# tingyu-c/TW-invoice-unet-ocr-llm

Hardware: AMD Instinct MI355X
Metric: invoice masks/sec at 512x512 bs256, 1/2/4/8 MI355X; IoU vs CPU ref (higher is better)
Workload: dtype bf16+fp16

## Files before the change

### tw-invoice-unet-ocr-llm_amd/csrc/unet_capi.cpp

```cpp
#include "unet_internal.h"
#include "unet_score.h"
#include "unet_loss.h"
#include "unet_head.h"
#include "../../include/unet_mi355x.h"

#include <dlfcn.h>

#include <algorithm>
#include <cmath>
#include <cstdio>
#include <cstdlib>
#include <cstring>
#include <list>
#include <map>
#include <string>
#include <thread>
#include <tuple>
#include <vector>

using namespace unet;

namespace {

thread_local std::string g_err;
// ... 87 lines not shown
  std::vector<void*> allocs;
  std::list<std::pair<std::tuple<int, int, int, int>, ResampleStore>> resample;
  uint8_t* pp_tmp = nullptr;
  size_t pp_tmp_bytes = 0;
  std::string labels[UNET_NUM_LAUNCHES];
  float thr_logit[kMaxClasses];
  hipEvent_t done = nullptr;
  hipStream_t last_stream = nullptr;
  bool pending = false;
  bool capturing = false;
  void* comm = nullptr;
  unsigned long long generation = 1;
  int ksplit_max = 32;
  int f32x3 = 0;
  int ksplit_force[21] = {};
  void* part = nullptr;
  int* box_sync = nullptr;
  int box_sync_n = 0;
  void* score = nullptr;
  size_t score_bytes = 0;
  void* loss = nullptr;
  size_t loss_bytes = 0;
  void* head = nullptr;
  size_t head_bytes = 0;
};

struct unet_graph {
  unet_handle* h = nullptr;
  hipGraph_t graph = nullptr;
  hipGraphExec_t exec = nullptr;
// ... 52 lines not shown
    {C3A, EPI_STORE, 2, B_(cat3), 512, B_(tA), 256},
    {C3B, EPI_STORE, 2, B_(tA), 256, B_(tB), 256},
    {19, EPI_UPSCATTER, 2, B_(tB), 256, B_(cat2), 256, 0, {}, 0, "u2", 128},
    {C2A, EPI_STORE, 1, B_(cat2), 256, B_(tA), 128},
    {C2B, EPI_STORE, 1, B_(tA), 128, B_(tB), 128, 0, {}, 0, "c7", 128},
    {20, EPI_UPSCATTER, 1, B_(tB), 128, B_(cat1), 128, 0, {}, 0, "u1", 64},
    {C1A, EPI_STORE, 0, B_(cat1), 128, B_(tA), 64, 0, {}, 0, "c8a", 64},
    {C1B, EPI_HEAD, 0, B_(tA), 64}};
#undef B_
static_assert(sizeof kLaunches / sizeof kLaunches[0] == UNET_NUM_LAUNCHES - 1, "one row per launch slot after the first");
const int kRingCfg[17] = {
    CFG_RING8_FUSED_IN,
    CFG_RING8_R128, CFG_RING8_R128, CFG_RING8_R128, CFG_RING8_R128, CFG_RING8_R128, CFG_RING8_R128,
    CFG_RING8_R128, CFG_RING8_R128, CFG_RING8_R128, CFG_RING8_R128, CFG_RING8_R128, CFG_RING8_R128,
    CFG_RING8_R128, CFG_RING8_R128,
    CFG_RING8_R64_T9, CFG_RING8_R64_WS};
const int kHaloCfg[17] = {
    CFG_HALO_R64_W8,
    CFG_HALO_R128, CFG_HALO_R128, CFG_HALO_R128, CFG_HALO_R64_W4, CFG_HALO_R128, CFG_HALO_R64_W4,
    CFG_HALO_R128, CFG_HALO_R128, CFG_HALO_R128, CFG_HALO_R128, CFG_HALO_R128, CFG_HALO_R128,
    CFG_HALO_R128, CFG_HALO_R128,
    CFG_HALO_R64_W4, CFG_HALO_R64_W8};

DType level_dtype(int dtype, int level) {
  switch (dtype) {
    case UNET_DTYPE_F32: case UNET_DTYPE_F32_EXACT: return DType::F32;
    case UNET_DTYPE_F16: return DType::F16;
    case UNET_DTYPE_MIXED: return level <= 1 ? DType::F16 : DType::BF16;
    default: return DType::BF16;
  }
}
// ... 70 lines not shown
  if (row.id >= 17) {
    if (!(row.id == 20 && h->fuse_up1)) st.L = &up_layer(h, row.id - 17, N);
    return st;
  }
  st.L = &h->L[row.id];
  if (row.id == C2B && h->fuse_up1) {
    st.r.epi = EPI_UPFUSE;
    st.r.out = nullptr;
    st.r.ldo = 0;
    st.r.out2 = &Buffers::cat1;
    st.r.ldo2 = 128;
  }
  if (row.id == D1B && cfg_fused_in(st.L->cfg)) st.r.id = -1;
  return st;
}
Split step_split(const unet_handle* h, const Step& st, int N, int H, int W) {
  return layer_split(h, st.r.id, *st.L, st.r.epi, N, H >> st.r.level, W >> st.r.level);
}

size_t split_bytes(const unet_handle* h, int N, int H, int W) {
  size_t m = 0;
  for (const Launch& row : kLaunches) {
    const Step st = resolve(h, row, N);
    const int ks = st.L ? step_split(h, st, N, H, W).ks : 1;
    if (ks > 1) m = std::max(m, (size_t)ks * N * (H >> row.level) * (W >> row.level) * st.L->ctot * 4);
  }
  return m;
}

Buffers plan(const unet_handle* h, int N, int H, int W) {
// ... 448 lines not shown
std::string layer_label(const Layer& L, int epi, Split sp = Split{}) {
  char buf[160];
  int cfg = L.cfg;
  if (sp.ks == 1 && sp.rows && cfg == CFG_TRING_R256) cfg = CFG_TRING_R128;
  if (sp.ks > 1) {
    Layer P = L;
    P.dto = P.dtq = L.dt;
    std::string part = layer_label(P, EPI_PARTIAL, Split{1, sp.rows});
    std::snprintf(buf, sizeof buf, " + splitk_reduce_kernel<%s, %s, %d>", tname(L.dto),
                  tname(epi == EPI_POOL ? L.dtq : L.dto), epi);
    return part + buf;
  }
  if (cfg_is_tring(cfg)) {
    std::snprintf(buf, sizeof buf, "convT_ring_kernel<%s, 8, %d, %d, %s>", tname(L.dt), cfg == CFG_TRING_R256 ? 4 : 3,
                  cfg == CFG_TRING_R256 ? 2 : 1, tname(L.dto));
  } else if (cfg_is_ring8(cfg)) {
    const int wst = cfg == CFG_RING8_R64_WS || cfg == CFG_RING8_FUSED_IN;
    const int rows = (sp.rows && cfg == CFG_RING8_R128) ? sp.rows : cfg_rows(cfg);
    std::snprintf(buf, sizeof buf, "conv3x3_ring8_kernel<%s, %d, %d, %d, %d, %d, %s, %s, %d, 0>", tname(L.dt),
                  rows / 16, ring_ns(cfg), epi, ring_tps(cfg), wst, tname(L.dto),
                  tname(epi == EPI_POOL ? L.dtq : L.dto), cfg == CFG_RING8_FUSED_IN ? 1 : 0);
  } else if (cfg_is_ring(cfg)) {
    std::snprintf(buf, sizeof buf, "conv3x3_ring_kernel<%s, 1, 4, %d, %d, %d, %d, %d, %s, %s, %d, %d>", tname(L.dt),
                  cfg_rows(cfg) / 16, ring_ns(cfg), epi, ring_tps(cfg), cfg == CFG_RING_FUSED_IN ? 1 : 0,
                  tname(L.dto), tname(epi == EPI_POOL ? L.dtq : L.dto), cfg_tile_h(cfg), cfg_tile_w(cfg));
  } else if (L.x3 == 3 || L.x3 == 4) {
    std::snprintf(buf, sizeof buf, L.x3 == 3 ? "conv3x3_x3s_kernel<%d>" : "conv3x3_x3w_kernel<%d>", epi);
  } else {
    const int wpx = cfg == CFG_HALO_R64_W8 ? 8 : 4, tc = cfg == CFG_HALO_R128 ? 8 : 4,
              ns = L.x3 == 2 ? 2 : cfg == CFG_HALO_R128 ? 2 : 3;
// ... 1 lines not shown
                  L.taps == 9 ? 3 : 1, epi, L.x3);
  }
  return buf;
}

void build_labels_at(const unet_handle* h, int N, int H, int W, std::string (&out)[UNET_NUM_LAUNCHES]) {
  const int C = h->cfg.n_channels;
  char buf[96];
  const DType t0 = h->L[D1B].dt;
  std::snprintf(buf, sizeof buf, t0 == DType::F32 ? "first_conv_kernel<%s, %d>" : "first_conv_mfma_kernel<%s, %d>",
                tname(t0), C);
  out[0] = cfg_fused_in(h->L[D1B].cfg) ? std::string("x_to_px4_kernel<") + tname(t0) + ">" : buf;
  int i = 1;
  for (const Launch& row : kLaunches) {
    const Step st = resolve(h, row, N);
    out[i++] = st.L ? layer_label(*st.L, st.r.epi, step_split(h, st, N, H, W)) : std::string();
  }
}
void build_labels(unet_handle* h) { build_labels_at(h, 0, 0, 0, h->labels); }

template <typename F>
void parse_pairs(const char* list, F each) {
  const std::string o(list ? list : "");
  for (size_t pos = 0, end; pos < o.size(); pos = end + 1) {
    end = std::min(o.find(',', pos), o.size());
    const std::string item = o.substr(pos, end - pos);
    const size_t colon = item.find(':');
    if (colon != std::string::npos)
      each(std::atoi(item.substr(0, colon).c_str()), std::atoi(item.substr(colon + 1).c_str()), item);
  }
}
void parse_overrides(const char* ov, int n, int* cfg_out, bool (*ok)(int)) {
  parse_pairs(ov, [&](int li, int c, const std::string& item) {
    if (li >= 0 && li < n && c >= 0 && c < cfg_limit() && ok(c)) cfg_out[li] = c;
    else std::fprintf(stderr, "unet_mi355x: ignoring configuration override '%s'\n", item.c_str());
  });
}

struct NcclId { char internal[UNET_COMM_ID_BYTES]; };
struct Rccl {
  void* lib = nullptr;
  int (*get_unique_id)(NcclId*) = nullptr;
  int (*comm_init_rank)(void**, int, NcclId, int) = nullptr;
  int (*all_gather)(const void*, void*, size_t, int, void*, hipStream_t) = nullptr;
  int (*comm_destroy)(void*) = nullptr;
  const char* (*error_string)(int) = nullptr;
};
const Rccl* rccl() {
  static Rccl r;
// ... 77 lines not shown
  for (const Launch& row : kLaunches) {
    if (row.id >= 17) continue;
    const int i = row.id;
    const bool pool = row.epi == EPI_POOL;
    Layer& L = h->L[i];
    L.cin = kLayerCh[i][0];
    L.cout = L.ctot = kLayerCh[i][1];
    L.taps = 9;
    L.dt = L.dto = level_dtype(cfg->dtype, row.level);
    L.dtq = level_dtype(cfg->dtype, row.level + 1);
    int c = cfgs[i];
    const bool ring = cfg_is_ring(c);
    if (cfg_fused_in(c) && (i != D1B || f32))
      c = cfg_is_ring8(c) ? (L.cout == 64 ? CFG_RING8_R64_T9 : CFG_RING8_R128)
                          : (L.cout == 64 ? CFG_RING_R64_T3 : CFG_RING_R128);
    if (c == CFG_RING8_R64_WS && (L.cin != 64 || f32)) c = L.cout == 64 ? CFG_RING8_R64_T9 : CFG_RING8_R128;
    if (c == CFG_RING8_R128 && (L.cout == 64 || f32)) c = CFG_RING8_R64_T9;
    if (c == CFG_RING_R64_W12 && f32) c = CFG_RING_R64_T3;
    if (cfg_rows(c) > L.cout || (i == C1B && cfg_rows(c) != 64))
      c = ring ? CFG_RING_R64_T3 : CFG_HALO_R64_W8;
    if (cfg_is_halo(c) && (L.dto != L.dt || (pool && L.dtq != L.dt))) c = L.cout == 64 || pool ? CFG_RING_R64_T3 : CFG_RING_R128;
    if (c == CFG_RING_R128 && pool) c = CFG_RING_R64_T3;
    if (h->f32x3 && f32) {
#ifndef UNET_X3_ONCE_MIN_CIN
#define UNET_X3_ONCE_MIN_CIN 128
#endif
      const bool once = h->f32x3 == 2 && L.cout % 128 == 0 && L.cin >= UNET_X3_ONCE_MIN_CIN && i != C1B;
      const bool wide = h->f32x3 == 2 && i == C1B;
      c = once ? CFG_HALO_R128 : wide ? CFG_HALO_X3W : CFG_HALO_R64_W4;
      L.x3 = once ? 3 : wide ? 4 : 2;
// ... 16 lines not shown
      U.x3 = 1;
      if (h->f32x3 == 2) {
        h->Us[i] = U;
        h->Us[i].cfg = CFG_HALO_R64_W4;
        h->Us[i].x3 = 2;
      }
    }
  }
  {
    const char* fz = std::getenv("UNET_MI355X_FUSE_UP1");
    const Layer &c2b = h->L[C2B], &u1 = h->U[3];
    h->fuse_up1 = !(fz && fz[0] == '0') && !f32 && (c2b.cfg == CFG_RING_R128 || c2b.cfg == CFG_RING8_R128) &&
                  u1.dt == c2b.dt && u1.dto == c2b.dto;
  }
  if (const char* ks = std::getenv("UNET_MI355X_KSPLIT")) h->ksplit_max = std::atoi(ks);
  parse_pairs(std::getenv("UNET_MI355X_KSPLIT_FORCE"), [&](int li, int ks, const std::string&) {
    if (li >= 0 && li < 21) h->ksplit_force[li] = ks;
  });
  build_labels(h);
  DeviceGuard g(cfg->device);
  const int rc = init_handle(h);
  if (rc) { delete h; return rc; }
  *out = h;
  return UNET_OK;
}

int unet_load_weights(unet_handle* h, const unet_tensor_view* t, int n) {
  if (!h || (!t && n)) return fail(UNET_EINVAL, "null argument");
  SD sd;
  for (int i = 0; i < n; ++i) {
// ... 130 lines not shown
  a.bias = L.b;
  a.zero = h->zero;
  a.out = out;
  a.out2 = out2;
  a.head_w = h->head_w;
  a.head_b = h->head_b;
  a.logits = logits;
  a.masks = static_cast<uint8_t*>(masks);
  a.N = N; a.H = H; a.W = W;
  a.Cin = L.cin; a.ldi = ldi;
  a.Ctot = L.ctot; a.Cout = L.cout;
  a.ldo = ldo; a.out_off = out_off; a.ldo2 = ldo2;
  a.ncls = h->cfg.n_classes;
  a.mask_kind = mask_kind;
  a.x3 = L.x3;
  if (epi == EPI_UPFUSE) {
    a.wgt = h->wf_c2b;
    a.bias2 = h->U[3].b;
  }
  if (cfg_fused_in(L.cfg)) {
    a.x0 = x0;
    a.w0p = h->w0r;
    a.b0 = h->b0;
    a.c0 = h->cfg.n_channels;
  }
  for (int i = 0; i < kMaxClasses; ++i) a.thr_logit[i] = h->thr_logit[i];
  a.tiles_x = (W + cfg_tile_w(L.cfg) - 1) / cfg_tile_w(L.cfg);
  a.tiles_y = (H + cfg_tile_h(L.cfg) - 1) / cfg_tile_h(L.cfg);
  a.n_ct = L.ctot / cfg_rows(L.cfg);
  const Split sp = layer_split(h, id, L, epi, N, H, W);
  int cfg = L.cfg;
  if (sp.ks == 1 && sp.rows) {
    a.src_br = cfg_rows(L.cfg);
    a.n_ct = L.ctot / sp.rows;
    if (L.cfg == CFG_TRING_R256) cfg = CFG_TRING_R128;
  }
  if (sp.ks > 1) {
    a.part = static_cast<float*>(h->part);
    a.ksplit = sp.ks;
    if (sp.rows) {
      a.src_br = cfg_rows(L.cfg);
      a.n_ct = L.ctot / sp.rows;
    }
    hipError_t e = launch_igemm(L.dt, L.dt, L.dt, L.cfg, L.taps, EPI_PARTIAL, a, s);
    if (e == hipSuccess) e = launch_splitk_reduce(L.dto, epi == EPI_POOL ? L.dtq : L.dto, epi, a, s);
    if (e != hipSuccess) return fail(UNET_EHIP, std::string("split-K igemm launch: ") + hipGetErrorString(e));
// ... 863 lines not shown
```

### tw-invoice-unet-ocr-llm_amd/csrc/unet_internal.h

```cpp
#pragma once
#include <hip/hip_runtime.h>
#include <cstdint>
#include <cstddef>

namespace unet {

enum class DType : int { F32 = 0, BF16 = 1, F16 = 2 };

inline size_t dtype_size(DType t) { return t == DType::F32 ? 4 : 2; }

enum Epi : int {
  EPI_STORE = 0,
  EPI_POOL = 1,
  EPI_HEAD = 2,
  EPI_UPSCATTER = 3,
  EPI_UPFUSE = 4,
  EPI_PARTIAL = 5
};

enum MaskKind : int { MASK_NONE = 0, MASK_U8 = 1, MASK_BITS = 2 };

constexpr int kMaxClasses = 4;

struct IgemmArgs {
// ... 12 lines not shown
  int Ctot;
  int Cout;
  int ldo, out_off, ldo2;
  int ncls, mask_kind;
  float thr_logit[kMaxClasses];
  int tiles_x, tiles_y, n_ct;
  const void* x0;
  const void* w0p;
  const float* b0;
  int c0;
  const float* bias2;
  float* part;
  int ksplit;
  int src_br;
  int x3;
};

struct FirstConvArgs {
  const float* x;
  const float* w;
  const void* wp;
  const float* b;
  void* out;
  int N, C, H, W;
};

__host__ __device__ constexpr int first_tap(int s) { return (int)((0xF8F5F2764310ull >> (4 * s)) & 15); }
__host__ __device__ constexpr int first_tap_addr(int s) { return (int)((0x885522764310ull >> (4 * s)) & 15); }

enum Cfg : int {
  CFG_HALO_R64_W4 = 0,
  CFG_HALO_R64_W8 = 1,
  CFG_HALO_R128 = 2,
  CFG_RING_R128 = 3,
  CFG_RING_R64_T3 = 4,
  CFG_RING_FUSED_IN = 5,
  CFG_TRING_R128 = 6,
  CFG_TRING_R256 = 7,
  CFG_RING8_R128 = 8,
  CFG_RING8_R64_T9 = 9,
  CFG_RING8_R64_WS = 10,
  CFG_RING8_FUSED_IN = 11,
  CFG_RING_R64_W12 = 12,
  CFG_HALO_X3W = 13,
  CFG_COUNT = 14
};
int cfg_rows(int cfg);
bool cfg_is_halo(int cfg);
bool cfg_is_ring(int cfg);
int ring_ns(int cfg);
int ring_tps(int cfg);
int cfg_tile_w(int cfg);
int cfg_tile_h(int cfg);
bool cfg_is_ring8(int cfg);
bool cfg_fused_in(int cfg);
bool cfg_is_tring(int cfg);
int cfg_limit();

hipError_t launch_igemm(DType t, DType to, DType tq, int cfg, int taps, int epi, const IgemmArgs& a,
                        hipStream_t s);
hipError_t launch_first_conv(DType t, const FirstConvArgs& a, hipStream_t s);
hipError_t launch_splitk_reduce(DType to, DType tq, int epi, const IgemmArgs& a, hipStream_t s);
hipError_t launch_x_to_px4(DType t, const void* x, int layout, int xdt, int N, int C, int H, int W, void* out,
                           hipStream_t s);
hipError_t launch_x_to_nchw_f32(const void* x, int layout, int xdt, int N, int C, int H, int W, float* out,
                                hipStream_t s);
hipError_t launch_nchw_to_nhwc(DType t, const float* x, int N, int C, int H, int W, void* out, hipStream_t s);
hipError_t launch_nhwc_to_nchw(DType t, const void* src, int N, int C, int H, int W, float* y, hipStream_t s);
hipError_t launch_nhwc_to_nchw_f32(DType t, const void* src, int N, int H, int W, int C, int ld,
                                   int choff, float* dst, hipStream_t s);
struct ResamplePlan {
  int ih, iw, oh, ow;
// ... 18 lines not shown
```

### tw-invoice-unet-ocr-llm_amd/csrc/unet_kernels.hip

```cpp
#include "unet_internal.h"

#include <algorithm>
#include <type_traits>

namespace unet {

typedef __bf16 bf16x8 __attribute__((ext_vector_type(8)));
typedef _Float16 f16x8 __attribute__((ext_vector_type(8)));
typedef float f32x4 __attribute__((ext_vector_type(4)));
typedef __attribute__((address_space(3))) void* lds_ptr_t;
typedef int frag_t __attribute__((ext_vector_type(4)));

int cfg_rows(int cfg) {
  switch (cfg % 16) {
    case CFG_HALO_R128: case CFG_RING_R128: case CFG_TRING_R128: case CFG_RING8_R128: return 128;
    case CFG_TRING_R256: return 256;
    default: return 64;
  }
}
bool cfg_is_halo(int cfg) {
  return cfg == CFG_HALO_R64_W4 || cfg == CFG_HALO_R64_W8 || cfg == CFG_HALO_R128 || cfg == CFG_HALO_X3W;
}
bool cfg_is_ring(int cfg) {
  cfg %= 16;
  return cfg == CFG_RING_R128 || cfg == CFG_RING_R64_T3 || cfg == CFG_RING_FUSED_IN || cfg == CFG_RING8_R128 ||
         cfg == CFG_RING8_R64_T9 || cfg == CFG_RING8_R64_WS || cfg == CFG_RING8_FUSED_IN || cfg == CFG_RING_R64_W12;
}
bool cfg_is_ring8(int cfg) {
  cfg %= 16;
  return cfg == CFG_RING8_R128 || cfg == CFG_RING8_R64_T9 || cfg == CFG_RING8_R64_WS || cfg == CFG_RING8_FUSED_IN;
}
int cfg_tile_w(int cfg) {
  return (cfg_is_ring8(cfg) || cfg % 16 == CFG_RING_R64_W12 || cfg == CFG_HALO_X3W) ? 32 : 16;
}
int cfg_tile_h(int cfg) { return cfg % 16 == CFG_RING_R64_W12 ? 12 : 16; }
bool cfg_fused_in(int cfg) { return cfg % 16 == CFG_RING_FUSED_IN || cfg % 16 == CFG_RING8_FUSED_IN; }
int ring_ns(int cfg) { return cfg % 16 == CFG_RING_R64_W12 ? 4 : (cfg % 16 == CFG_RING8_R64_T9 ? 2 : 3); }
int ring_tps(int cfg) {
  cfg %= 16;
  if (cfg == CFG_RING8_R64_T9) return 9;
  return (cfg == CFG_RING_R64_T3 || cfg == CFG_RING_FUSED_IN || cfg == CFG_RING8_R128 || cfg == CFG_RING8_R64_WS ||
          cfg == CFG_RING8_FUSED_IN) ? 3 : 1;
}
int cfg_limit() {
#ifdef UNET_ABLATION
  return CFG_COUNT + 16 * 10;
#else
  return CFG_RING_R64_W12;
#endif
}
bool cfg_is_tring(int cfg) { return cfg == CFG_TRING_R128 || cfg == CFG_TRING_R256; }

template <typename T> struct Elem;
template <> struct Elem<float> { static constexpr int BKE = 32; };
template <> struct Elem<__bf16> { static constexpr int BKE = 64; };
// ... 86 lines not shown
  d[0] = __builtin_bit_cast(uint4, lo);
  d[1] = __builtin_bit_cast(uint4, hi);
}
template <>
__device__ __forceinline__ void store16<_Float16>(_Float16* dst, const float (&v)[16]) {
  f16x8 lo, hi;
#pragma unroll
  for (int i = 0; i < 8; ++i) { lo[i] = (_Float16)v[i]; hi[i] = (_Float16)v[8 + i]; }
  uint4* d = reinterpret_cast<uint4*>(dst);
  d[0] = __builtin_bit_cast(uint4, lo);
  d[1] = __builtin_bit_cast(uint4, hi);
}

__device__ __forceinline__ int swz_store_off(int q) { return 8 * ((q & 1) * 2 + (q >> 1)); }
template <typename T>
__device__ __forceinline__ void store64_grouped(T* grp, const float (&v)[16]) {
  if constexpr (sizeof(T) == 4) {
    store16<T>(grp + 16 * ((threadIdx.x & 63) >> 4), v);
  } else {
    typedef T t8 __attribute__((ext_vector_type(8)));
    t8 lo, hi;
#pragma unroll
    for (int i = 0; i < 8; ++i) { lo[i] = (T)v[i]; hi[i] = (T)v[8 + i]; }
    uint4 x = __builtin_bit_cast(uint4, lo), y = __builtin_bit_cast(uint4, hi);
    uint4 xs, ys;
#pragma unroll
    for (int i = 0; i < 4; ++i) {
      const auto r = __builtin_amdgcn_permlane32_swap(x[i], y[i], false, false);
      xs[i] = r[0];
      ys[i] = r[1];
    }
    T* dst = grp + swz_store_off((threadIdx.x & 63) >> 4);
    *reinterpret_cast<uint4*>(dst) = xs;
    *reinterpret_cast<uint4*>(dst + 32) = ys;
  }
}

__device__ __forceinline__ void glds16(const void* src, char* lds_dst) {
  const uint32_t lds_addr = __builtin_amdgcn_readfirstlane(
      static_cast<uint32_t>(reinterpret_cast<uintptr_t>((lds_ptr_t)lds_dst)));
  unsigned keep;
  asm volatile(
      "s_mov_b32 %0, m0\n\t"
      "s_mov_b32 m0, %2\n\t"
      "s_nop 0\n\t"
      "global_load_lds_dwordx4 %1, off\n\t"
// ... 339 lines not shown
    if (k + 1 < NT) load(k + 1, b ^ 1);
#pragma unroll
    for (int t = 0; t < TC; ++t)
#pragma unroll
      for (int p = 0; p < TP; ++p)
        mfma_frag<T>(acc[t][p], __builtin_bit_cast(uint4, fa[b][t]), __builtin_bit_cast(uint4, fb[b][p]));
    if (k + 1 < NT) {
#pragma unroll
      for (int i = 0; i < NR; ++i) {
        __builtin_amdgcn_sched_group_barrier(0x008, NM / NR, 0);
        __builtin_amdgcn_sched_group_barrier(0x100, 1, 0);
      }
    } else {
      __builtin_amdgcn_sched_group_barrier(0x008, NM, 0);
    }
    if (k == 0) mid();
  }
}

template <typename T, int TC, int TP, int NT, int ABL = 0, typename Mid = NoMid>
__device__ __forceinline__ void mfma_taps_astream(f32x4 (&acc)[TC][TP], const char* const (&hs)[NT],
                                                  const char* const (&ws)[NT], const int (&prow)[TP], Mid mid = Mid{}) {
  static_assert(TC >= TP && TC >= 3, "B prefetch spread over the row groups");
  frag_t ar[3], fb[2][TP];
  frag_t rf = {};
  if constexpr (ABL == 3) rf = *reinterpret_cast<const frag_t*>(hs[0] + prow[0]);
  auto ldsread = [&](const char* p) {
    if constexpr (ABL == 3) {
      frag_t v = rf;
      asm volatile("" : "+v"(v));
      return v;
// ... 11 lines not shown
  for (int k = 0; k < NT; ++k) {
#pragma unroll
    for (int t = 0; t < TC; ++t) {
      const int j = k * TC + t;
      if (j + 2 < NT * TC) ar[(j + 2) % 3] = lda(j + 2);
      if (k + 1 < NT && t < TP) fb[(k + 1) & 1][t] = ldsread(hs[k + 1] + prow[t]);
      const frag_t af = ar[j % 3];
#pragma unroll
      for (int p = 0; p < TP; ++p) {
        if constexpr (ABL == 2) asm volatile("" ::"v"(af), "v"(fb[k & 1][p]));
        else mfma_frag<T>(acc[t][p], __builtin_bit_cast(uint4, af), __builtin_bit_cast(uint4, fb[k & 1][p]));
      }
      if (j + 2 < NT * TC) __builtin_amdgcn_sched_group_barrier(0x100, 1, 0);
      if (k + 1 < NT && t < TP) __builtin_amdgcn_sched_group_barrier(0x100, 1, 0);
      __builtin_amdgcn_sched_group_barrier(0x008, TP, 0);
      if (j == 1) mid();
    }
  }
}

template <typename T, int WR, int WPX, int TCW, int NS, int KT, int X3 = 0>
struct HaloGeom {
  static constexpr int NW = WR * WPX;
  static constexpr int TC = TCW;
  static constexpr int TP = 16 / WPX;
  static constexpr int BR = WR * 16 * TC;
  static constexpr int BKE = Elem<T>::BKE;
  static constexpr int PAD = KT == 3 ? 1 : 0;
  static constexpr int HWD = 16 + 2 * PAD;
  static constexpr int NPIX = HWD * HWD;
  static constexpr int NTAP = KT * KT;
// ... 1678 lines not shown
          conv_epilogue<TO, TQ, TP, EPI, TW, ABL == 6 ? 1 : 2, 1>(a, *reinterpret_cast<const f32x4(*)[4][TP]>(&acc[4 * h]), n,
                                                               ty * 16, tx * TW, wp * TP, ct * BR + 64 * h, bias_s + 64 * h,
                                                               headw_s, headb_s);
        } else {
          conv_epilogue<TO, TQ, TP, EPI, TW, 0, 1>(a, *reinterpret_cast<const f32x4(*)[4][TP]>(&acc[4 * h]), n, ty * 16,
                                                   tx * TW, wp * TP, ct * BR + 64 * h, bias_s + 64 * h, headw_s,
                                                   headb_s);
        }
      }
      init_acc_bias(0, TC);
      ++item;
    }
  }
}

template <typename T, int TCW, int NS, int EPI, int TPS, int WST, typename TO, typename TQ, int HS = 0, int ABL = 0>
static hipError_t launch_ring8(const IgemmArgs& a, hipStream_t s) {
  using G = Ring8Geom<T, TCW, NS, TPS, WST, HS>;
  if constexpr (HS != 0) {
    if (a.Cin != 2 * G::BKE || a.c0 < 1 || a.c0 > 3 || !a.x0 || !a.w0p || !a.b0) return hipErrorInvalidValue;
  }
  if (a.tiles_y != (a.H + 15) / 16 || a.tiles_x != (a.W + G::TW - 1) / G::TW) return hipErrorInvalidValue;
  if (a.Cin % G::BKE || a.Ctot % G::BR || a.n_ct != a.Ctot / G::BR) return hipErrorInvalidValue;
  if (WST && (9 / TPS) * (a.Cin / G::BKE) > G::WST_STEPS) return hipErrorInvalidValue;
  const int KS = EPI == EPI_PARTIAL ? a.ksplit : 1;
  if (KS < 1 || a.Cin % (G::BKE * KS) || (EPI == EPI_PARTIAL && !a.part)) return hipErrorInvalidValue;
  constexpr bool fine = TCW == 4 && NS == 3 && TPS == 3 && WST == 0 && HS == 0 && EPI != EPI_UPFUSE;
  if (a.src_br && (!(EPI == EPI_PARTIAL || fine) || a.src_br % G::BR || a.Ctot % a.src_br)) return hipErrorInvalidValue;
  const int n_mt = a.N * a.tiles_y * a.tiles_x * KS;
  int n_slots = kNumCUs / a.n_ct;
  n_slots -= n_slots % KS;
  if (n_slots < KS) n_slots = KS;
  if (n_slots > n_mt) n_slots = n_mt;
  hipLaunchKernelGGL((conv3x3_ring8_kernel<T, TCW, NS, EPI, TPS, WST, TO, TQ, HS, ABL>), dim3(a.n_ct * n_slots), dim3(512),
                     0, s, a);
  return hipGetLastError();
}

template <typename T, int TCW, int NS, int WRW = 1, typename TO = T>
__global__ __launch_bounds__(256 * WRW, WRW == 1 ? 2 : 1) void convT_ring_kernel(const IgemmArgs a) {
  constexpr int NW = 4 * WRW, TC = TCW, TP = 4, BR = 16 * TC * WRW, BKE = 64 / (int)sizeof(T);
  constexpr int WI = BR / (16 * NW);
  constexpr int BI = 256 / (16 * NW);
  constexpr int ASLOT = BR * 64, BSLOT = 256 * 64, SLOT = ASLOT + BSLOT;
  static_assert((NS == 3 || NS == 4) && TC % 4 == 0, "ring depth / row tile");
  static_assert(NS * SLOT + BR * 4 <= 160 * 1024 / (WRW == 1 ? 2 : 1), "blocks per CU");
  __shared__ __attribute__((aligned(16))) char lds[NS * SLOT];
  __shared__ __attribute__((aligned(16))) float bias_s[BR];
// ... 422 lines not shown
#ifdef UNET_ABLATION
    case CFG_RING_R64_W12:
      if constexpr (sizeof(T) == 2) return launch_ring<T, 1, 4, 4, 4, EPI, 1, 0, TO, TQ, 0, 12, 32>(a, s);
      break;
#endif
    case CFG_RING_FUSED_IN:
      if constexpr (sizeof(T) == 2 && EPI == EPI_POOL) return launch_ring<T, 1, 4, 4, 3, EPI, 3, 1, TO, TQ>(a, s);
      break;
    case CFG_RING8_R128:
      if constexpr (EPI != EPI_HEAD && sizeof(T) == 2) {
        if (a.src_br == 128) return launch_ring8<T, 4, 3, EPI, 3, 0, TO, TQ>(a, s);
        return launch_ring8<T, 8, 3, EPI, 3, 0, TO, TQ>(a, s);
      }
      break;
    case CFG_RING8_R64_T9: if constexpr (EPI != EPI_PARTIAL) return launch_ring8<T, 4, 2, EPI, 9, 0, TO, TQ>(a, s); break;
    case CFG_RING8_R64_WS: return launch_ring8<T, 4, 3, EPI, 3, 1, TO, TQ>(a, s);
    case CFG_RING8_FUSED_IN:
      if constexpr (sizeof(T) == 2 && EPI == EPI_POOL) return launch_ring8<T, 4, 3, EPI, 3, 1, TO, TQ, 1>(a, s);
      break;
    default: break;
  }
  return hipErrorInvalidValue;
  }
}

template <typename T, typename TO, int EPI = EPI_UPSCATTER>
static hipError_t launch_up(int cfg, const IgemmArgs& a, hipStream_t s) {
  if constexpr (EPI == EPI_PARTIAL) {
    if (cfg == CFG_HALO_R128) return launch_halo<T, 1, 4, 8, 2, EPI_PARTIAL, 1>(a, s);
    if constexpr (sizeof(T) == 4)
// ... 537 lines not shown
```

Baseline: 3527.

## Add paired-tile ring8 conv kernel sharing weight loads across two tiles

```diff
diff --git a/tw-invoice-unet-ocr-llm_amd/csrc/unet_capi.cpp b/tw-invoice-unet-ocr-llm_amd/csrc/unet_capi.cpp
--- a/tw-invoice-unet-ocr-llm_amd/csrc/unet_capi.cpp
+++ b/tw-invoice-unet-ocr-llm_amd/csrc/unet_capi.cpp
@@ -125,6 +125,7 @@
   int ksplit_max = 32;
   int f32x3 = 0;
   int ksplit_force[21] = {};
+  int walkers = 0;
   void* part = nullptr;
   int* box_sync = nullptr;
   int box_sync_n = 0;
@@ -207,7 +208,7 @@
     CFG_RING8_R128, CFG_RING8_R128, CFG_RING8_R128, CFG_RING8_R128, CFG_RING8_R128, CFG_RING8_R128,
     CFG_RING8_R128, CFG_RING8_R128, CFG_RING8_R128, CFG_RING8_R128, CFG_RING8_R128, CFG_RING8_R128,
     CFG_RING8_R128, CFG_RING8_R128,
-    CFG_RING8_R64_T9, CFG_RING8_R64_WS};
+    CFG_RING8_R64_PAIR, CFG_RING8_R64_WS};
 const int kHaloCfg[17] = {
     CFG_HALO_R64_W8,
     CFG_HALO_R128, CFG_HALO_R128, CFG_HALO_R128, CFG_HALO_R64_W4, CFG_HALO_R128, CFG_HALO_R64_W4,
@@ -308,6 +309,14 @@
   if (row.id == D1B && cfg_fused_in(st.L->cfg)) st.r.id = -1;
   return st;
 }
+int run_cfg(const unet_handle* h, const Layer& L, int N, int Hl, int Wl) {
+  if (L.cfg != CFG_RING8_R64_PAIR || N <= 0) return L.cfg;
+  const int n_ct = L.ctot / cfg_rows(L.cfg);
+  const long long n_mt = (long long)N * ((Hl + cfg_tile_h(L.cfg) - 1) / cfg_tile_h(L.cfg)) *
+                         ((Wl + cfg_tile_w(L.cfg) - 1) / cfg_tile_w(L.cfg));
+  const long long walkers = ring8_walkers(n_ct, (int)n_mt, 1, h->walkers);
+  return n_mt >= 2 * walkers ? (int)CFG_RING8_R64_PAIR : (int)CFG_RING8_R64_T9;
+}
 Split step_split(const unet_handle* h, const Step& st, int N, int H, int W) {
   return layer_split(h, st.r.id, *st.L, st.r.epi, N, H >> st.r.level, W >> st.r.level);
 }
@@ -786,6 +795,9 @@
   if (cfg_is_tring(cfg)) {
     std::snprintf(buf, sizeof buf, "convT_ring_kernel<%s, 8, %d, %d, %s>", tname(L.dt), cfg == CFG_TRING_R256 ? 4 : 3,
                   cfg == CFG_TRING_R256 ? 2 : 1, tname(L.dto));
+  } else if (cfg == CFG_RING8_R64_PAIR) {
+    std::snprintf(buf, sizeof buf, "conv3x3_ring8_kernel<%s, 4, 2, %d, 9, 0, %s, %s, 0, 0, 1>", tname(L.dt), epi, tname(L.dto),
+                  tname(L.dto));
   } else if (cfg_is_ring8(cfg)) {
     const int wst = cfg == CFG_RING8_R64_WS || cfg == CFG_RING8_FUSED_IN;
     const int rows = (sp.rows && cfg == CFG_RING8_R128) ? sp.rows : cfg_rows(cfg);
@@ -817,7 +829,13 @@
   int i = 1;
   for (const Launch& row : kLaunches) {
     const Step st = resolve(h, row, N);
-    out[i++] = st.L ? layer_label(*st.L, st.r.epi, step_split(h, st, N, H, W)) : std::string();
+    if (!st.L) {
+      out[i++] = std::string();
+      continue;
+    }
+    Layer L = *st.L;
+    if (row.id < 17) L.cfg = run_cfg(h, L, N, H >> row.level, W >> row.level);
+    out[i++] = layer_label(L, st.r.epi, step_split(h, st, N, H, W));
   }
 }
 void build_labels(unet_handle* h) { build_labels_at(h, 0, 0, 0, h->labels); }
@@ -835,7 +853,7 @@
 }
 void parse_overrides(const char* ov, int n, int* cfg_out, bool (*ok)(int)) {
   parse_pairs(ov, [&](int li, int c, const std::string& item) {
-    if (li >= 0 && li < n && c >= 0 && c < cfg_limit() && ok(c)) cfg_out[li] = c;
+    if (li >= 0 && li < n && c >= 0 && (c < cfg_limit() || c == CFG_RING8_R64_PAIR) && ok(c)) cfg_out[li] = c;
     else std::fprintf(stderr, "unet_mi355x: ignoring configuration override '%s'\n", item.c_str());
   });
 }
@@ -943,6 +961,7 @@
     if (cfg_fused_in(c) && (i != D1B || f32))
       c = cfg_is_ring8(c) ? (L.cout == 64 ? CFG_RING8_R64_T9 : CFG_RING8_R128)
                           : (L.cout == 64 ? CFG_RING_R64_T3 : CFG_RING_R128);
+    if (c == CFG_RING8_R64_PAIR && (L.cout != 64 || L.cin % 64 || f32 || row.epi != EPI_STORE)) c = L.cout == 64 ? CFG_RING8_R64_T9 : CFG_RING8_R128;
     if (c == CFG_RING8_R64_WS && (L.cin != 64 || f32)) c = L.cout == 64 ? CFG_RING8_R64_T9 : CFG_RING8_R128;
     if (c == CFG_RING8_R128 && (L.cout == 64 || f32)) c = CFG_RING8_R64_T9;
     if (c == CFG_RING_R64_W12 && f32) c = CFG_RING_R64_T3;
@@ -989,6 +1008,7 @@
                   u1.dt == c2b.dt && u1.dto == c2b.dto;
   }
   if (const char* ks = std::getenv("UNET_MI355X_KSPLIT")) h->ksplit_max = std::atoi(ks);
+  if (const char* wk = std::getenv("UNET_MI355X_WALKERS")) h->walkers = std::max(0, std::atoi(wk));
   parse_pairs(std::getenv("UNET_MI355X_KSPLIT_FORCE"), [&](int li, int ks, const std::string&) {
     if (li >= 0 && li < 21) h->ksplit_force[li] = ks;
   });
@@ -1149,6 +1169,7 @@
   a.ncls = h->cfg.n_classes;
   a.mask_kind = mask_kind;
   a.x3 = L.x3;
+  a.walkers = h->walkers;
   if (epi == EPI_UPFUSE) {
     a.wgt = h->wf_c2b;
     a.bias2 = h->U[3].b;
@@ -1164,7 +1185,7 @@
   a.tiles_y = (H + cfg_tile_h(L.cfg) - 1) / cfg_tile_h(L.cfg);
   a.n_ct = L.ctot / cfg_rows(L.cfg);
   const Split sp = layer_split(h, id, L, epi, N, H, W);
-  int cfg = L.cfg;
+  int cfg = run_cfg(h, L, N, H, W);
   if (sp.ks == 1 && sp.rows) {
     a.src_br = cfg_rows(L.cfg);
     a.n_ct = L.ctot / sp.rows;
diff --git a/tw-invoice-unet-ocr-llm_amd/csrc/unet_internal.h b/tw-invoice-unet-ocr-llm_amd/csrc/unet_internal.h
--- a/tw-invoice-unet-ocr-llm_amd/csrc/unet_internal.h
+++ b/tw-invoice-unet-ocr-llm_amd/csrc/unet_internal.h
@@ -50,6 +50,7 @@
   int ksplit;
   int src_br;
   int x3;
+  int walkers;
 };
 
 struct FirstConvArgs {
@@ -79,7 +80,8 @@
   CFG_RING8_FUSED_IN = 11,
   CFG_RING_R64_W12 = 12,
   CFG_HALO_X3W = 13,
-  CFG_COUNT = 14
+  CFG_RING8_R64_PAIR = 14,
+  CFG_COUNT = 15
 };
 int cfg_rows(int cfg);
 bool cfg_is_halo(int cfg);
@@ -92,6 +94,7 @@
 bool cfg_fused_in(int cfg);
 bool cfg_is_tring(int cfg);
 int cfg_limit();
+int ring8_walkers(int n_ct, int n_mt, int ks, int cap);
 
 hipError_t launch_igemm(DType t, DType to, DType tq, int cfg, int taps, int epi, const IgemmArgs& a,
                         hipStream_t s);
diff --git a/tw-invoice-unet-ocr-llm_amd/csrc/unet_kernels.hip b/tw-invoice-unet-ocr-llm_amd/csrc/unet_kernels.hip
--- a/tw-invoice-unet-ocr-llm_amd/csrc/unet_kernels.hip
+++ b/tw-invoice-unet-ocr-llm_amd/csrc/unet_kernels.hip
@@ -24,21 +24,26 @@
 bool cfg_is_ring(int cfg) {
   cfg %= 16;
   return cfg == CFG_RING_R128 || cfg == CFG_RING_R64_T3 || cfg == CFG_RING_FUSED_IN || cfg == CFG_RING8_R128 ||
-         cfg == CFG_RING8_R64_T9 || cfg == CFG_RING8_R64_WS || cfg == CFG_RING8_FUSED_IN || cfg == CFG_RING_R64_W12;
+         cfg == CFG_RING8_R64_T9 || cfg == CFG_RING8_R64_WS || cfg == CFG_RING8_FUSED_IN || cfg == CFG_RING_R64_W12 ||
+         cfg == CFG_RING8_R64_PAIR;
 }
 bool cfg_is_ring8(int cfg) {
   cfg %= 16;
-  return cfg == CFG_RING8_R128 || cfg == CFG_RING8_R64_T9 || cfg == CFG_RING8_R64_WS || cfg == CFG_RING8_FUSED_IN;
+  return cfg == CFG_RING8_R128 || cfg == CFG_RING8_R64_T9 || cfg == CFG_RING8_R64_WS || cfg == CFG_RING8_FUSED_IN ||
+         cfg == CFG_RING8_R64_PAIR;
 }
 int cfg_tile_w(int cfg) {
   return (cfg_is_ring8(cfg) || cfg % 16 == CFG_RING_R64_W12 || cfg == CFG_HALO_X3W) ? 32 : 16;
 }
 int cfg_tile_h(int cfg) { return cfg % 16 == CFG_RING_R64_W12 ? 12 : 16; }
 bool cfg_fused_in(int cfg) { return cfg % 16 == CFG_RING_FUSED_IN || cfg % 16 == CFG_RING8_FUSED_IN; }
-int ring_ns(int cfg) { return cfg % 16 == CFG_RING_R64_W12 ? 4 : (cfg % 16 == CFG_RING8_R64_T9 ? 2 : 3); }
+int ring_ns(int cfg) {
+  cfg %= 16;
+  return cfg == CFG_RING_R64_W12 ? 4 : (cfg == CFG_RING8_R64_T9 || cfg == CFG_RING8_R64_PAIR ? 2 : 3);
+}
 int ring_tps(int cfg) {
   cfg %= 16;
-  if (cfg == CFG_RING8_R64_T9) return 9;
+  if (cfg == CFG_RING8_R64_T9 || cfg == CFG_RING8_R64_PAIR) return 9;
   return (cfg == CFG_RING_R64_T3 || cfg == CFG_RING_FUSED_IN || cfg == CFG_RING8_R128 || cfg == CFG_RING8_R64_WS ||
           cfg == CFG_RING8_FUSED_IN) ? 3 : 1;
 }
@@ -155,22 +160,30 @@
 
 __device__ __forceinline__ int swz_store_off(int q) { return 8 * ((q & 1) * 2 + (q >> 1)); }
 template <typename T>
+__device__ __forceinline__ void cast64_grouped(const float (&v)[16], uint4& x, uint4& y) {
+  typedef T t8 __attribute__((ext_vector_type(8)));
+  t8 lo, hi;
+#pragma unroll
+  for (int i = 0; i < 8; ++i) { lo[i] = (T)v[i]; hi[i] = (T)v[8 + i]; }
+  x = __builtin_bit_cast(uint4, lo);
+  y = __builtin_bit_cast(uint4, hi);
+}
+__device__ __forceinline__ void swap64_grouped(const uint4& x, const uint4& y, uint4& xs, uint4& ys) {
+#pragma unroll
+  for (int i = 0; i < 4; ++i) {
+    const auto r = __builtin_amdgcn_permlane32_swap(x[i], y[i], false, false);
+    xs[i] = r[0];
+    ys[i] = r[1];
+  }
+}
+template <typename T>
 __device__ __forceinline__ void store64_grouped(T* grp, const float (&v)[16]) {
   if constexpr (sizeof(T) == 4) {
     store16<T>(grp + 16 * ((threadIdx.x & 63) >> 4), v);
   } else {
-    typedef T t8 __attribute__((ext_vector_type(8)));
-    t8 lo, hi;
-#pragma unroll
-    for (int i = 0; i < 8; ++i) { lo[i] = (T)v[i]; hi[i] = (T)v[8 + i]; }
-    uint4 x = __builtin_bit_cast(uint4, lo), y = __builtin_bit_cast(uint4, hi);
-    uint4 xs, ys;
-#pragma unroll
-    for (int i = 0; i < 4; ++i) {
-      const auto r = __builtin_amdgcn_permlane32_swap(x[i], y[i], false, false);
-      xs[i] = r[0];
-      ys[i] = r[1];
-    }
+    uint4 x, y, xs, ys;
+    cast64_grouped<T>(v, x, y);
+    swap64_grouped(x, y, xs, ys);
     T* dst = grp + swz_store_off((threadIdx.x & 63) >> 4);
     *reinterpret_cast<uint4*>(dst) = xs;
     *reinterpret_cast<uint4*>(dst + 32) = ys;
@@ -540,7 +553,8 @@
     } else {
       __builtin_amdgcn_sched_group_barrier(0x008, NM, 0);
     }
-    if (k == 0) mid();
+    if constexpr (std::is_invocable_v<Mid&, int>) mid(k);
+    else if (k == 0) mid();
   }
 }
 
@@ -582,7 +596,11 @@
       if (j + 2 < NT * TC) __builtin_amdgcn_sched_group_barrier(0x100, 1, 0);
       if (k + 1 < NT && t < TP) __builtin_amdgcn_sched_group_barrier(0x100, 1, 0);
       __builtin_amdgcn_sched_group_barrier(0x008, TP, 0);
-      if (j == 1) mid();
+      if constexpr (std::is_invocable_v<Mid&, int>) {
+        if (t == TC - 1) mid(k);
+      } else if (j == 1) {
+        mid();
+      }
     }
   }
 }
@@ -2291,6 +2309,272 @@
   }
 }
 
+template <typename T, int TCW, int NS, int EPI, int TPS, int WST, typename TO, typename TQ, int HS, int ABL, int PAIR>
+__global__ __launch_bounds__(512, 2) void conv3x3_ring8_kernel(const IgemmArgs a) {
+  static_assert(TCW == 4 && NS == 2 && EPI == EPI_STORE && TPS == 9 && WST == 0 && HS == 0 && ABL == 0 && PAIR == 1 &&
+                    sizeof(T) == 2,
+                "the pair ring: 16-bit, 64 rows, one chunk per step, two weight slots, plain stores");
+  using G = Ring8Geom<T, TCW, NS, TPS, WST, HS>;
+  constexpr int NW = G::NW, TW = G::TW, TC = G::TC, TP = G::TP, BR = G::BR, BKE = G::BKE;
+  constexpr int HWD = G::HWD, HP = G::HP, HI = G::HI, HALO_BYTES = G::HALO_BYTES;
+  constexpr int WSLOT = G::WSLOT, SLOT = G::SLOT, PIECES = G::PIECES, WOFF = G::WOFF;
+  static_assert(G::LDS_BYTES <= 160 * 1024, "LDS");
+  __shared__ __attribute__((aligned(16))) char lds[G::LDS_BYTES];
+  float* bias_s = reinterpret_cast<float*>(lds + G::PARAM_OFF);
+
+  const int tid = threadIdx.x;
+  const int wave = __builtin_amdgcn_readfirstlane(tid >> 6);
+  const uint32_t lds0 = lds_addr_of(lds);
+  const int lane = tid & 63;
+  const int wp = wave;
+
+  int ct, slot;
+  {
+    const int nb = gridDim.x, q = nb >> 3, r = nb & 7;
+    const int b = blockIdx.x, x = b & 7, k = b >> 3;
+    const int bid = (x < r ? x * (q + 1) : r * (q + 1) + (x - r) * q) + k;
+    ct = bid % a.n_ct;
+    slot = bid / a.n_ct;
+  }
+  const int n_slots = gridDim.x / a.n_ct;
+  const int n_mt = a.N * a.tiles_y * a.tiles_x;
+  if (slot >= n_mt) return;
+  const int items = (n_mt - slot + n_slots - 1) / n_slots;
+  const int H = a.H, W = a.W;
+  const int nch = a.Cin / BKE;
+
+  const char* wblk = reinterpret_cast<const char*>(a.wgt) + (size_t)ct * nch * SLOT;
+  const uint32_t wlane = (lane >> 2) * 64 + (((lane & 3) ^ ((lane >> 3) & 3)) << 4);
+  const char* in = reinterpret_cast<const char*>(a.in);
+  const char* zero = reinterpret_cast<const char*>(a.zero);
+
+  auto tile_of = [&](int i, int& n, int& ty, int& tx) {
+    int mt = slot + i * n_slots;
+    tx = mt % a.tiles_x;
+    mt /= a.tiles_x;
+    ty = mt % a.tiles_y;
+    n = mt / a.tiles_y;
+  };
+  uint32_t hoff[HI];
+#pragma unroll
+  for (int j = 0; j < HI; ++j) {
+    const int row = (wave * HI + j) * 16 + (lane >> 2);
+    const int hy = row / HWD, hx = row - (row / HWD) * HWD;
+    hoff[j] = (uint32_t)(hy * W + hx) * (uint32_t)(a.ldi * (int)sizeof(T)) + (((lane & 3) ^ (hx & 3)) << 4);
+  }
+  struct HaloTile {
+    const char* org;
+    uint32_t ok;
+  };
+  auto halo_tile = [&](int i) {
+    int n, ty, tx;
+    tile_of(i, n, ty, tx);
+    HaloTile t;
+    t.org = in + ((long long)(n * H + ty * 16 - 1) * W + (tx * TW - 1)) * a.ldi * (long long)sizeof(T);
+    t.ok = 0;
+    int l4 = lane >> 2;
+    asm volatile("" : "+v"(l4));
+#pragma unroll
+    for (int j = 0; j < HI; ++j) {
+      const int row = (wave * HI + j) * 16 + l4;
+      const int hy = row / HWD, hx = row - (row / HWD) * HWD;
+      const int iy = ty * 16 + hy - 1, ix = tx * TW + hx - 1;
+      if (row < HP && (unsigned)iy < (unsigned)H && (unsigned)ix < (unsigned)W) t.ok |= 1u << j;
+    }
+    return t;
+  };
+  auto issue_halo = [&](const HaloTile& t, int c, int buf) {
+    const uint32_t dst = lds0 + buf * HALO_BYTES + wave * HI * 1024;
+#pragma unroll
+    for (int j = 0; j < HI; ++j) {
+      uint32_t o = hoff[j];
+      asm volatile("" : "+v"(o));
+      const char* src = (t.ok >> j) & 1 ? t.org + o : zero + (o & 48);
+      glds16_s(src + c * 64, dst + j * 1024);
+    }
+  };
+  auto issue_w = [&](int c, int dst_slot) {
+    const char* src = wblk + (size_t)c * SLOT;
+    const uint32_t dst = lds0 + WOFF + dst_slot * SLOT;
+#pragma unroll
+    for (int k = 0; k < (PIECES + NW - 1) / NW; ++k) {
+      const int j = wave + k * NW;
+      if (PIECES % NW == 0 || j < PIECES) glds16_sv(src + j * 1024, wlane, dst + j * 1024);
+    }
+  };
+  f32x4 accA[TC][TP], accB[TC][TP];
+  const int col = lane & 15, q = lane >> 4;
+  auto init_acc_bias = [&](f32x4 (&acc)[TC][TP]) {
+#pragma unroll
+    for (int t = 0; t < TC; ++t) {
+      const f32x4 b4 = *reinterpret_cast<const f32x4*>(bias_s + 16 * q + 4 * t);
+#pragma unroll
+      for (int p = 0; p < TP; ++p) acc[t][p] = b4;
+    }
+  };
+  int prow[TP];
+#pragma unroll
+  for (int p = 0; p < TP; ++p) {
+    int py, px;
+    pix_of_w<TW>((wp * TP + p) * 16 + col, py, px);
+    prow[p] = (py * HWD + px) * 64;
+  }
+  const int px_lane = col & 7;
+  const int wpos = (q ^ ((col >> 1) & 3)) << 4;
+  const char* wrow = lds + WOFF + col * 64 + wpos;
+  static_assert(TW / 8 == TP, "one row pair per wave");
+  int opy, opx;
+  pix_of_w<TW>(wp * TP * 16 + col, opy, opx);
+  const uint32_t poff = ((uint32_t)(opy * W + opx) * (uint32_t)a.ldo + (uint32_t)swz_store_off(q)) * (uint32_t)sizeof(TO);
+  const int pstep = 8 * a.ldo * (int)sizeof(TO);
+  auto out_origin = [&](int n, int ty, int tx) {
+    return reinterpret_cast<char*>(a.out) +
+           (((long long)(n * H + ty * 16) * W + tx * TW) * a.ldo + a.out_off + ct * BR) * (long long)sizeof(TO);
+  };
+  auto cast_tile = [&](const f32x4 (&acc)[TC][TP], uint4 (&pk)[TP][2]) __attribute__((always_inline)) {
+#pragma unroll
+    for (int p = 0; p < TP; ++p) {
+      float v[16];
+#pragma unroll
+      for (int t = 0; t < TC; ++t)
+#pragma unroll
+        for (int e = 0; e < 4; ++e) v[t * 4 + e] = relu_nan(acc[t][p][e]);
+      uint4 x, y;
+      cast64_grouped<TO>(v, x, y);
+      unsigned d[8] = {x[0], x[1], x[2], x[3], y[0], y[1], y[2], y[3]};
+      asm volatile("" : "+v"(d[0]), "+v"(d[1]), "+v"(d[2]), "+v"(d[3]), "+v"(d[4]), "+v"(d[5]), "+v"(d[6]), "+v"(d[7]));
+      pk[p][0] = uint4{d[0], d[1], d[2], d[3]};
+      pk[p][1] = uint4{d[4], d[5], d[6], d[7]};
+    }
+  };
+  auto store_group = [&](const uint4 (&pk)[TP][2], int p, char* org, int ty, int tx) __attribute__((always_inline)) {
+    uint4 xs, ys;
+    swap64_grouped(pk[p][0], pk[p][1], xs, ys);
+    if (ty * 16 + opy < H && tx * TW + 8 * p + opx < W) {
+      char* d = org + p * pstep + poff;
+      *reinterpret_cast<uint4*>(d) = xs;
+      *reinterpret_cast<uint4*>(d + 32 * sizeof(TO)) = ys;
+    }
+  };
+  auto store_tile = [&](const f32x4 (&acc)[TC][TP], int n, int ty, int tx) __attribute__((always_inline)) {
+    uint4 pk[TP][2];
+    cast_tile(acc, pk);
+    char* const org = out_origin(n, ty, tx);
+#pragma unroll
+    for (int p = 0; p < TP; ++p) store_group(pk, p, org, ty, tx);
+  };
+  auto taps = [&](f32x4 (&acc)[TC][TP], int par, auto hook) {
+    int hb = par, ws = par;
+    asm volatile("" : "+s"(hb), "+s"(ws));
+    const char* hs9[9];
+    const char* ws9[9];
+#pragma unroll
+    for (int k = 0; k < 9; ++k) {
+      const int dy = k / 3, dx = k % 3;
+      hs9[k] = lds + hb * HALO_BYTES + (dy * HWD + dx) * 64 + ((q ^ ((px_lane + dx) & 3)) << 4);
+      ws9[k] = wrow + ws * SLOT + k * WSLOT;
+    }
+    mfma_taps_astream<T, TC, TP, 9>(acc, hs9, ws9, prow, hook);
+  };
+
+  HaloTile hsA = halo_tile(0), hsB = hsA;
+  issue_halo(hsA, 0, 0);
+  issue_w(0, 0);
+  for (int i = tid; i < BR; i += 64 * NW) bias_s[i] = a.bias[ct * BR + i];
+  wait_vm_barrier<0>();
+  init_acc_bias(accA);
+  init_acc_bias(accB);
+
+  int i = 0;
+  for (; i + 1 < items; i += 2) {
+    int nA, tyA, txA, nB, tyB, txB;
+    tile_of(i, nA, tyA, txA);
+    tile_of(i + 1, nB, tyB, txB);
+    char* const orgA = out_origin(nA, tyA, txA);
+    hsB = halo_tile(i + 1);
+    const bool more = i + 2 < items;
+    uint4 pkA[TP][2];
+    auto four_steps = [&](int c, auto lastc) __attribute__((always_inline)) {
+      constexpr bool last = decltype(lastc)::value;
+      issue_w(c + 1, 1);
+      issue_halo(hsA, c + 1, 1);
+      taps(accA, 0, NoMid{});
+      wait_vm_barrier<0>();
+      issue_halo(hsB, c, 0);
+      taps(accA, 1, NoMid{});
+      if constexpr (last) cast_tile(accA, pkA);
+      wait_vm_barrier<0>();
+      issue_halo(hsB, c + 1, 1);
+      if constexpr (last) {
+        taps(accB, 0, [&](int k) __attribute__((always_inline)) {
+#pragma unroll
+          for (int p = 0; p < TP; ++p)
+            if (k == p + 1) store_group(pkA, p, orgA, tyA, txA);
+        });
+      } else {
+        taps(accB, 0, NoMid{});
+      }
+      wait_vm_barrier<0>();
+      if constexpr (!last) {
+        issue_w(c + 2, 0);
+        issue_halo(hsA, c + 2, 0);
+      } else if (more) {
+        issue_w(0, 0);
+        hsA = halo_tile(i + 2);
+        issue_halo(hsA, 0, 0);
+      }
+      taps(accB, 1, NoMid{});
+      wait_vm_barrier<0>();
+    };
+    for (int c = 0; c + 2 < nch; c += 2) four_steps(c, std::false_type{});
+    four_steps(nch - 2, std::true_type{});
+    store_tile(accB, nB, tyB, txB);
+    init_acc_bias(accA);
+    init_acc_bias(accB);
+  }
+  if (i < items) {
+    int n, ty, tx;
+    tile_of(i, n, ty, tx);
+    for (int c = 0; c < nch; c += 2) {
+      issue_w(c + 1, 1);
+      issue_halo(hsA, c + 1, 1);
+      taps(accA, 0, NoMid{});
+      wait_vm_barrier<0>();
+      if (c + 2 < nch) {
+        issue_w(c + 2, 0);
+        issue_halo(hsA, c + 2, 0);
+      }
+      taps(accA, 1, NoMid{});
+      wait_vm_barrier<0>();
+    }
+    store_tile(accA, n, ty, tx);
+  }
+}
+
+int ring8_walkers(int n_ct, int n_mt, int ks, int cap) {
+  int n_slots = kNumCUs / n_ct;
+  if (cap > 0 && n_slots > cap) n_slots = cap;
+  n_slots -= n_slots % ks;
+  if (n_slots < ks) n_slots = ks;
+  if (n_slots > n_mt) n_slots = n_mt;
+  return n_slots;
+}
+
+template <typename T, typename TO, typename TQ>
+static hipError_t launch_ring8_pair(const IgemmArgs& a, hipStream_t s) {
+  using G = Ring8Geom<T, 4, 2, 9, 0, 0>;
+  if (a.tiles_y != (a.H + 15) / 16 || a.tiles_x != (a.W + G::TW - 1) / G::TW) return hipErrorInvalidValue;
+  if (a.Cin % (2 * G::BKE) || a.Ctot % G::BR || a.n_ct != a.Ctot / G::BR || a.src_br) return hipErrorInvalidValue;
+  const long long pstride = (long long)a.ldi * (long long)sizeof(T);
+  if (pstride % 64 || (18LL * a.W + G::HWD) * pstride >= (1LL << 32)) return hipErrorInvalidValue;
+  if ((16LL * a.W + G::TW) * a.ldo * (long long)sizeof(TO) >= (1LL << 32)) return hipErrorInvalidValue;
+  const int n_mt = a.N * a.tiles_y * a.tiles_x;
+  const int n_slots = ring8_walkers(a.n_ct, n_mt, 1, a.walkers);
+  hipLaunchKernelGGL((conv3x3_ring8_kernel<T, 4, 2, EPI_STORE, 9, 0, TO, TQ, 0, 0, 1>), dim3(a.n_ct * n_slots), dim3(512),
+                     0, s, a);
+  return hipGetLastError();
+}
+
 template <typename T, int TCW, int NS, int EPI, int TPS, int WST, typename TO, typename TQ, int HS = 0, int ABL = 0>
 static hipError_t launch_ring8(const IgemmArgs& a, hipStream_t s) {
   using G = Ring8Geom<T, TCW, NS, TPS, WST, HS>;
@@ -2305,10 +2589,7 @@
   constexpr bool fine = TCW == 4 && NS == 3 && TPS == 3 && WST == 0 && HS == 0 && EPI != EPI_UPFUSE;
   if (a.src_br && (!(EPI == EPI_PARTIAL || fine) || a.src_br % G::BR || a.Ctot % a.src_br)) return hipErrorInvalidValue;
   const int n_mt = a.N * a.tiles_y * a.tiles_x * KS;
-  int n_slots = kNumCUs / a.n_ct;
-  n_slots -= n_slots % KS;
-  if (n_slots < KS) n_slots = KS;
-  if (n_slots > n_mt) n_slots = n_mt;
+  const int n_slots = ring8_walkers(a.n_ct, n_mt, KS, a.walkers);
   hipLaunchKernelGGL((conv3x3_ring8_kernel<T, TCW, NS, EPI, TPS, WST, TO, TQ, HS, ABL>), dim3(a.n_ct * n_slots), dim3(512),
                      0, s, a);
   return hipGetLastError();
@@ -2761,6 +3042,9 @@
       }
       break;
     case CFG_RING8_R64_T9: if constexpr (EPI != EPI_PARTIAL) return launch_ring8<T, 4, 2, EPI, 9, 0, TO, TQ>(a, s); break;
+    case CFG_RING8_R64_PAIR:
+      if constexpr (EPI == EPI_STORE && sizeof(T) == 2 && std::is_same<TO, TQ>::value) return launch_ring8_pair<T, TO, TQ>(a, s);
+      break;
     case CFG_RING8_R64_WS: return launch_ring8<T, 4, 3, EPI, 3, 1, TO, TQ>(a, s);
     case CFG_RING8_FUSED_IN:
       if constexpr (sizeof(T) == 2 && EPI == EPI_POOL) return launch_ring8<T, 4, 3, EPI, 3, 1, TO, TQ, 1>(a, s);
```

Result: no change. 3534, median of 6 (+0.2%).
